# boschresearch/what-matters-for-meta-learning

Hardware: AMD Instinct MI355X
Metric: meta-tasks/sec (fwd+bwd), ANP ShapeNet1D 15+15-shot 16-task batch (higher is better)
Workload: dtype f32

## Files before the change

### what-matters-for-meta-learning_amd/csrc/conv_tc.h

```cpp
#pragma once
#include "common.h"

#ifndef MLHOT_HOSTSIM
namespace mlhot {
#ifdef MLHOT_TS
namespace tf { extern __device__ long long* g_ts_dev; }
#endif
namespace c2 {

typedef float f32x4_t __attribute__((ext_vector_type(4)));

constexpr int CIN = 32, COUT = 48;
constexpr int NT = 768;
#ifndef C12_NT_STORE
#define C12_NT_STORE 0
#endif
#ifndef C12_M1_LANE0
#define C12_M1_LANE0 0
#endif
#ifndef C12_EARLY_PIXELS
#define C12_EARLY_PIXELS 0
#endif
constexpr int RS = 65, ROWS = 9, PS = ROWS * RS;
constexpr int PATCH_FLOATS = CIN * PS;
// ... 199 lines not shown
  return iy1 >= 0 ? (((size_t)img * 64 + iy1) * 4 + cg) * M1_REC : (size_t)n_img * 4096;
}

struct Conv1Tile {
  float a[3];
  f32x4_t c0, c1;
};
__device__ __forceinline__ void c1t_mfma(Conv1Tile& t, const Conv1W& cw, int i) {
  const int ks = i >> 1;
  const f32x4_t zero = {0.f, 0.f, 0.f, 0.f};
  if (i & 1) t.c1 = mfma4(t.a[ks], cw.b[ks][1], ks == 0 ? zero : t.c1);
  else t.c0 = mfma4(t.a[ks], cw.b[ks][0], ks == 0 ? zero : t.c0);
}
template <bool MASK>
__device__ __forceinline__ void c1t_post(Conv1Tile& t, int r, float* d, unsigned* __restrict__ mrec) {
  if (!MASK) {
    d[r] = __int_as_float(max(__float_as_int(t.c0[r]), 0));
    d[16 * PS + r] = __int_as_float(max(__float_as_int(t.c1[r]), 0));
    return;
  }
  const bool p0 = t.c0[r] > 0.f, p1 = t.c1[r] > 0.f;
  d[r] = p0 ? t.c0[r] : 0.f;
  d[16 * PS + r] = p1 ? t.c1[r] : 0.f;
  if (MASK) {
    const unsigned long long b0 = __builtin_amdgcn_ballot_w64(p0), b1 = __builtin_amdgcn_ballot_w64(p1);
    *reinterpret_cast<uint4*>(mrec + 4 * r) = make_uint4((unsigned)b0, (unsigned)(b0 >> 32), (unsigned)b1, (unsigned)(b1 >> 32));
  }
}
constexpr int CS = 34, CROW = RS * CS, CPATCH = ROWS * CROW;
static_assert(2 * CPATCH * 4 <= 160 * 1024, "LDS");
__device__ __forceinline__ float* c1t_dst_cl(float* patch, int t, int lr, int lq) {
  return patch + ((t >> 2) * RS + 1 + 16 * (t & 3) + 4 * lq) * CS + lr;
}
template <bool MASK>
__device__ __forceinline__ void c1t_post_cl(Conv1Tile& t, int r, float* d, unsigned* __restrict__ mrec, bool lane0 = true) {
  const bool p0 = t.c0[r] > 0.f, p1 = t.c1[r] > 0.f;
  d[r * CS] = p0 ? t.c0[r] : 0.f;
  d[r * CS + 16] = p1 ? t.c1[r] : 0.f;
  if (MASK) {
    const unsigned long long b0 = __builtin_amdgcn_ballot_w64(p0), b1 = __builtin_amdgcn_ballot_w64(p1);
#if C12_M1_LANE0
    if (lane0)
#endif
    *reinterpret_cast<uint4*>(mrec + 4 * r) = make_uint4((unsigned)b0, (unsigned)(b0 >> 32), (unsigned)b1, (unsigned)(b1 >> 32));
  }
}
__device__ __forceinline__ void patch_zero_pad_cl(float* patch, int tid) {
  for (int i = tid; i < ROWS * CS; i += NT) patch[(i / CS) * CROW + i % CS] = 0.f;
}

__device__ __forceinline__ float* c1t_dst(float* patch, int t, int lr, int lq) {
  return patch + lr * PS + (t >> 2) * RS + 1 + 16 * (t & 3) + 4 * lq;
}
__device__ __forceinline__ unsigned* c1t_rec(unsigned* __restrict__ m1, int tile, int tt, int n_img) {
  return m1 + m1_record(tile >> 3, 8 * (tile & 7) - 1 + (tt >> 2), tt & 3, n_img);
}
template <bool MASK, bool CL = false>
__device__ __forceinline__ void conv1_tile(const Conv1A& ca, const Conv1W& cw, int j, float* patch, int tile, int wave, int lane,
                                           unsigned* __restrict__ m1, int n_img) {
  const int lr = lane & 15, lq = lane >> 4, tt = wave + 12 * j;
  Conv1Tile t;
#pragma unroll
  for (int ks = 0; ks < 3; ++ks) t.a[ks] = ca.a[j][ks];
#pragma unroll
  for (int i = 0; i < 6; ++i) c1t_mfma(t, cw, i);
  float* d = CL ? c1t_dst_cl(patch, tt, lr, lq) : c1t_dst(patch, tt, lr, lq);
  unsigned* mrec = MASK ? c1t_rec(m1, tile, tt, n_img) : nullptr;
#pragma unroll
  for (int r = 0; r < 4; ++r) {
    if (CL) c1t_post_cl<MASK>(t, r, d, mrec); else c1t_post<MASK>(t, r, d, mrec);
  }
}

__device__ __forceinline__ float strip_line(const ImgSrc& x, int tile, int li) {
  li = min(li, 75);
  const int row = min(max(16 * (tile & 7) - 3 + (li >> 2), 0), 127);
  return x.img(tile >> 3)[row * 128 + 32 * (li & 3)];
}

__global__ __launch_bounds__(NT) void conv12_fwd_pool_kernel(const ImgSrc x, const float* __restrict__ w1, const float* __restrict__ b1,
                                                             const float* __restrict__ w, const float* __restrict__ bias,
                                                             float* __restrict__ p2, uint8_t* __restrict__ amax,
                                                             unsigned* __restrict__ m1, int n_img, int dbg) {
  __shared__ __attribute__((aligned(16))) float patch2[2 * CPATCH];
  static_assert(COUT * W2_LD <= 2 * CPATCH, "weight staging area");
  const int tid = threadIdx.x, lane = tid & 63, wave = __builtin_amdgcn_readfirstlane(tid >> 6);
  const int nt = wave % 3, pg = wave / 3, rp = pg >> 1, ch = pg & 1;
  const int lr = lane & 15, lq = lane >> 4;
  const int n = nt * 16 + lr;
  const int phase = __builtin_amdgcn_readfirstlane(wave >> 2);
#ifdef MLHOT_TS
  if (tf::g_ts_dev && blockIdx.x == 0 && tid == 0) tf::g_ts_dev[502] = clock64();
#endif

  conv2w_stage<NT>(patch2, w, tid);
  __syncthreads();
  float wr[72];
#pragma unroll
  for (int ks = 0; ks < 72; ++ks) wr[ks] = patch2[n * W2_LD + (8 * ((ks & 7) >> 1) + 2 * lq + (ks & 1)) * 9 + (ks >> 3)];
  const float bn = bias[n];
  __syncthreads();
  Conv1W cw;
  conv1w_load(cw, w1, b1, lr, lq);
  Conv1Lane cl;
  conv1lane_init(cl, wave, lr, lq);

  patch_zero_pad_cl(patch2, tid);
  patch_zero_pad_cl(patch2 + CPATCH, tid);
  const int ntiles = n_img * 8;
  int tile = first_tile<8>(blockIdx.x, gridDim.x);
#ifdef MLHOT_TS
  long long ts_c0 = clock64(), ts_w0 = wall_clock64();
  if (tf::g_ts_dev && blockIdx.x == 0 && tid == 0) tf::g_ts_dev[503] = ts_c0;
#endif
  if (tile < ntiles) {
    Conv1A ca;
    conv1a_fetch(ca, x, tile, wave, lr, lq);
#pragma unroll
    for (int j = 0; j < 3; ++j) conv1_tile<true, true>(ca, cw, j, patch2, tile, wave, lane, m1, n_img);
  }
  __syncthreads();
  const int aoff = ((4 * rp) * RS + 2 * (16 * ch + lr)) * CS + 2 * lq;
  int cur = 0;
  float warm = 0.f;
  if (wave < 2 && tile + (int)gridDim.x < ntiles) warm = strip_line(x, tile + (int)gridDim.x, tid);
  for (; tile < ntiles; tile += gridDim.x, cur ^= 1) {
    const float* ab = patch2 + cur * CPATCH + aoff;
    float* nb = patch2 + (cur ^ 1) * CPATCH;
    const int next = tile + (int)gridDim.x < ntiles ? tile + (int)gridDim.x : tile;

#ifdef MLHOT_TS
    const bool tsb = tf::g_ts_dev && blockIdx.x == 0 && (tile - (int)blockIdx.x) / (int)gridDim.x == 6;
    if (tsb && (lane == 0)) tf::g_ts_dev[400 + wave * 4 + 0] = clock64();
#endif
    f32x4_t acc0 = {0.f, 0.f, 0.f, 0.f}, acc1 = {0.f, 0.f, 0.f, 0.f};
    typedef float f32x2_t __attribute__((ext_vector_type(2)));
    constexpr int RDP = 2;
    auto aread = [&](int p, int row2) {
      const int tap = p >> 2, ky = tap / 3, kx = tap % 3, m = p & 3;
      return *reinterpret_cast<const f32x2_t*>(ab + (ky + row2) * CROW + kx * CS + 8 * m);
    };
    f32x2_t xa0[RDP], xa1[RDP];
#pragma unroll
    for (int d = 0; d < RDP; ++d) { xa0[d] = aread(d, 0); xa1[d] = aread(d, 2); }
    Conv1Tile ct;
    float bnw = bn;
#pragma unroll
    for (int ks = 0; ks < 72; ++ks) {
      if (ks % 24 == 0) set_wave_prio((phase + ks / 24) % 3);
      acc0 = mfma4(xa0[(ks >> 1) % RDP][ks & 1], wr[ks], acc0);
      acc1 = mfma4(xa1[(ks >> 1) % RDP][ks & 1], wr[ks], acc1);
      if ((ks & 1) && (ks >> 1) + RDP < 36) { xa0[(ks >> 1) % RDP] = aread((ks >> 1) + RDP, 0); xa1[(ks >> 1) % RDP] = aread((ks >> 1) + RDP, 2); }
      const int j = ks / 22, s = ks - 22 * j;
      if (j < 3) {
        const int tt = wave + 12 * j;
#if C12_EARLY_PIXELS
        if (j == 0 && s < 3) ct.a[s] = conv1a_pixel_load(cl, x, next, 0, s);
        else if (j < 2 && s >= 12 && s < 15) ct.a[s - 12] = conv1a_pixel_load(cl, x, next, j + 1, s - 12);
#else
        if (s < 3) ct.a[s] = conv1a_pixel_load(cl, x, next, j, s);
#endif
        if (s >= 5 && s < 8) ct.a[s - 5] = conv1a_pixel_blend(ct.a[s - 5], cl, next, j, s - 5, wave >> 2);
        else if (s >= 8 && s < 14) c1t_mfma(ct, cw, s - 8);
#ifdef C12_KNOCK_M1
        else if (s >= 15 && s < 19) c1t_post_cl<false>(ct, s - 15, c1t_dst_cl(nb, tt, lr, lq), nullptr);
#else
        else if (s >= 15 && s < 19) c1t_post_cl<true>(ct, s - 15, c1t_dst_cl(nb, tt, lr, lq), c1t_rec(m1, next, tt, n_img), lane == 0);
#endif
      }
      if (ks == 7) bnw = __builtin_fmaf(warm, 0.f, bn);
      if (ks == 48 && wave < 2) warm = strip_line(x, next + (int)gridDim.x < ntiles ? next + (int)gridDim.x : next, tid);
      __builtin_amdgcn_sched_barrier(0);
    }
#ifdef MLHOT_TS
    if (tsb && (lane == 0)) tf::g_ts_dev[400 + wave * 4 + 1] = clock64();
#endif
    const int img = tile >> 3, band = tile & 7;
    float pv[2]; unsigned pa[2];
#pragma unroll
    for (int j = 0; j < 2; ++j) {
      const float c0 = fmaxf(acc0[2 * j] + bnw, 0.f), c1 = fmaxf(acc0[2 * j + 1] + bnw, 0.f);
      const float c2v = fmaxf(acc1[2 * j] + bnw, 0.f), c3 = fmaxf(acc1[2 * j + 1] + bnw, 0.f);
      float best = c0; unsigned which = 0;
      if (c1 > best) { best = c1; which = 1; }
      if (c2v > best) { best = c2v; which = 2; }
      if (c3 > best) { best = c3; which = 3; }
      pv[j] = best; pa[j] = which;
    }
    const size_t o = (((size_t)img * COUT + n) * 16 + 2 * band + rp) * 16 + 8 * ch + 2 * lq;
#if C12_NT_STORE
    __builtin_nontemporal_store(f32x2_t{pv[0], pv[1]}, reinterpret_cast<f32x2_t*>(p2 + o));
    __builtin_nontemporal_store((unsigned short)(pa[0] | (pa[1] << 8)), reinterpret_cast<unsigned short*>(amax + o));
#else
    *reinterpret_cast<float2*>(p2 + o) = make_float2(pv[0], pv[1]);
    *reinterpret_cast<unsigned short*>(amax + o) = (unsigned short)(pa[0] | (pa[1] << 8));
#endif
#ifdef MLHOT_TS
    if (tsb && (lane == 0)) tf::g_ts_dev[400 + wave * 4 + 2] = clock64();
#endif
    __syncthreads();
#ifdef MLHOT_TS
    if (tsb && (lane == 0)) tf::g_ts_dev[400 + wave * 4 + 3] = clock64();
#endif
  }
#ifdef MLHOT_TS
  if (tf::g_ts_dev && blockIdx.x == 0 && threadIdx.x == 0) {
    tf::g_ts_dev[500] = clock64() - ts_c0; tf::g_ts_dev[501] = wall_clock64() - ts_w0;
  }
#endif
}

__device__ __forceinline__ int wg_px(int e) { return (e & 7) + ((e >> 2) & 8); }
__device__ __forceinline__ int wg_pyl(int e) { return (e >> 6) & 1; }
__device__ __forceinline__ int wg_co(int e) { return ((e >> 3) & 3) + 4 * (e >> 7); }
__global__ __launch_bounds__(NT) void conv12_wgrad_kernel(const ImgSrc x, const float* __restrict__ w1, const float* __restrict__ b1,
                                                          const float* __restrict__ dp2, const float* __restrict__ p2,
                                                          const uint8_t* __restrict__ amax, float* __restrict__ slab_w,
                                                          float* __restrict__ slab_b, int n_img, int dbg) {
  __shared__ float lds[PATCH_FLOATS + DYT_FLOATS];
  float* patch = lds;
  float* dyt = lds + PATCH_FLOATS;
  const int tid = threadIdx.x, lane = tid & 63, wave = __builtin_amdgcn_readfirstlane(tid >> 6);
  const int mg = wave % 6, ph = wave / 6;
  const int lr = lane & 15, lq = lane >> 4;
  const bool cact = !(dbg & 1);
  Conv1W cw;
  conv1w_load(cw, w1, b1, lr, lq);

  f32x4_t acc[3][3];
#pragma unroll
  for (int i = 0; i < 3; ++i)
#pragma unroll
    for (int j = 0; j < 3; ++j) acc[i][j] = f32x4_t{0.f, 0.f, 0.f, 0.f};
  float bsum[2] = {0.f, 0.f};

  patch_zero_pad(patch, tid);
  const int ntiles = n_img * 8;
  Conv1A ca;
  float cdp[2], cp[2]; unsigned cam[2];
  auto cells_fetch = [&](int t) {
    const int img = t >> 3, band = t & 7;
#pragma unroll
    for (int j = 0; j < 2; ++j) {
      const int e = tid + j * NT, px = wg_px(e), pyl = wg_pyl(e), co = wg_co(e);
      const size_t o = (((size_t)img * COUT + co) * 16 + 2 * band + pyl) * 16 + px;
      cdp[j] = dp2[o]; cp[j] = p2[o]; cam[j] = amax[o];
    }
  };
  int tile = first_tile<8>(blockIdx.x, gridDim.x);
  Conv1Lane cl;
  conv1lane_init(cl, wave, lr, lq);
  if (tile < ntiles) { if (cact) conv1a_fetch_fast(ca, cl, x, tile, wave); cells_fetch(tile); }
  int aoff[3];
#pragma unroll
  for (int i = 0; i < 3; ++i) {
    const int mt = 3 * mg + i, tap = mt >> 1, ky = tap / 3, kx = tap % 3;
    aoff[i] = (16 * (mt & 1) + lr) * PS + ky * RS + kx + 2 * (8 * lq);
  }
  const int boff = (8 * lq) * DS + lr;

  for (; tile < ntiles; tile += gridDim.x) {
#ifdef MLHOT_TS
    const bool tsb = tf::g_ts_dev && blockIdx.x == 0 && lane == 0 && (tile - first_tile<8>(0, gridDim.x)) / (int)gridDim.x == 6;
#define WG_STAMP(i) do { if (tsb) tf::g_ts_dev[360 + wave * 5 + (i)] = clock64(); } while (0)
#else
#define WG_STAMP(i) do { } while (0)
#endif
    WG_STAMP(0);
    __syncthreads();
    WG_STAMP(1);
    if (cact) {
#pragma unroll
      for (int j = 0; j < 3; ++j) conv1_tile<false>(ca, cw, j, patch, tile, wave, lane, nullptr, n_img);
    }
#pragma unroll
    for (int j = 0; j < 2; ++j) {
      const int e = tid + j * NT, px = wg_px(e), pyl = wg_pyl(e), co = wg_co(e);
      const float g = cp[j] > 0.f ? cdp[j] : 0.f;
      bsum[j] += g;
#pragma unroll
      for (int q = 0; q < 4; ++q)
        dyt[((2 * pyl + (q >> 1)) * 32 + 2 * px + (q & 1)) * DS + co] = (cam[j] == (unsigned)q) ? g : 0.f;
    }
    WG_STAMP(2);
    __syncthreads();
    WG_STAMP(3);
    if (tile + (int)gridDim.x < ntiles) { if (cact) conv1a_fetch_fast(ca, cl, x, tile + gridDim.x, wave); cells_fetch(tile + gridDim.x); }

#pragma unroll
    for (int s = 0; s < 16; ++s) {
      const int orow_l = s >> 3, oxb = s & 7;
      float a[3], b[3];
      const int arow = (2 * (2 * ph + orow_l)) * RS + 2 * oxb;
#pragma unroll
      for (int i = 0; i < 3; ++i) a[i] = patch[aoff[i] + arow];
      const int brow = ((2 * ph + orow_l) * 32 + oxb) * DS;
#pragma unroll
      for (int j = 0; j < 3; ++j) b[j] = dyt[boff + brow + 16 * j];
#pragma unroll
      for (int i = 0; i < 3; ++i)
#pragma unroll
        for (int j = 0; j < 3; ++j) acc[i][j] = mfma4(a[i], b[j], acc[i][j]);
    }
    WG_STAMP(4);
  }

  __syncthreads();
  if (ph == 1) {
#pragma unroll
    for (int i = 0; i < 3; ++i)
#pragma unroll
      for (int j = 0; j < 3; ++j)
#pragma unroll
        for (int r = 0; r < 4; ++r) lds[((mg * 9 + i * 3 + j) * 4 + r) * 64 + lane] = acc[i][j][r];
  }
  __syncthreads();
  if (ph == 0) {
    float* sw = slab_w + (size_t)blockIdx.x * (COUT * CIN * 9 + COUT);
#pragma unroll
    for (int i = 0; i < 3; ++i) {
// ... 250 lines not shown
```

### what-matters-for-meta-learning_amd/csrc/encoder.h

```cpp
#pragma once
#include "common.h"
#include "foreach.h"
#include "igemm.h"
#include "ops_direct.h"
#include "problems.h"
#include "favor.h"
#include "conv_tc.h"
#include "conv_split.h"
#include "conv3_tc.h"
#include "enc_linear.h"
#include "../../include/mlhot.h"

namespace mlhot {

struct Options { int conv2_tc; int tail_fused; int materialize_a1; int dbg; int tail_spec; int conv2_split; int conv3_bwd_merged; };
extern Options g_opt;
enum TailSpec : int {
  TAIL_SPEC_FWD_A = 1,
  TAIL_SPEC_FWD_B = 2,
  TAIL_SPEC_FWD_C = 4,
  TAIL_SPEC_BWD_C = 8,
  TAIL_SPEC_BWD_B = 16,
  TAIL_SPEC_BWD_A = 32,
  TAIL_SPEC_ENC_FOLD = 64,
  TAIL_SPEC_LOSS = 128,
  TAIL_SPEC_BWD_B_SPLIT = 512,
  TAIL_SPEC_BWD_C_WG2 = 1024,
  TAIL_SPEC_BWD_A_WG2 = 2048,
  TAIL_SPEC_WG4 = 4096,
  TAIL_SPEC_DEFAULT = TAIL_SPEC_FWD_A | TAIL_SPEC_FWD_B | TAIL_SPEC_FWD_C | TAIL_SPEC_BWD_C | TAIL_SPEC_BWD_B | TAIL_SPEC_BWD_A |
                      TAIL_SPEC_ENC_FOLD | TAIL_SPEC_LOSS | TAIL_SPEC_BWD_B_SPLIT | TAIL_SPEC_BWD_C_WG2 | TAIL_SPEC_BWD_A_WG2 |
                      TAIL_SPEC_WG4,
};
static_assert(TAIL_SPEC_DEFAULT == 7935, "the numeric values are public: tests, scripts and MLHOT_OPTS pass numbers");
constexpr int C2_GRID = 256;

struct EncSaved {
  float* a1; float* p2; uint8_t* am2; float* a3; unsigned* m1; bool ok; size_t bytes;
};
inline EncSaved enc_saved_carve(int n, void* base, size_t cap) {
  Arena a(base, cap);
  EncSaved s;
  s.a1 = a.take<float>((size_t)n * 32 * 64 * 64);
  s.p2 = a.take<float>((size_t)n * 48 * 16 * 16);
  s.am2 = a.take<uint8_t>((size_t)n * 48 * 16 * 16);
  s.a3 = a.take<float>((size_t)n * 4096);
  s.m1 = a.take<unsigned>((size_t)n * 64 * 64 + 16);
  s.ok = a.ok; s.bytes = a.off + 256;
  return s;
}
inline size_t enc_saved_bytes(int n) { return enc_saved_carve(n, nullptr, 0).bytes; }

inline int enc_lin_split(int n) { (void)n; return 32; }
inline int enc_linw_split(int n) { return n >= 64 ? 4 : 1; }
inline int conv3w_split(int n) { int s = n / 4; return s < 1 ? 1 : (s > 128 ? 128 : s); }
inline int conv2w_split(int n) { int s = n / 2; return s < 1 ? 1 : (s > 240 ? 240 : s); }
inline int conv1w_split(int n) { int s = n * 2; return s > 1024 ? 1024 : s; }

struct EncScratch {
  float* a2;
  float* slab;
  float* dy3;
  float* dp2;
  float* dy1;
  bool ok; size_t bytes;
};
inline size_t enc_slab_floats(int n, int dim_w) {
  size_t m = (size_t)enc_lin_split(n) * n * dim_w;
  size_t v;
  v = (size_t)enc_linw_split(n) * dim_w * 4097; if (v > m) m = v;
  v = (size_t)conv3w_split(n) * 64 * 433;       if (v > m) m = v;
  v = (size_t)conv2w_split(n) * 48 * 289;       if (v > m) m = v;
  v = (size_t)conv1w_split(n) * 32 * 10;        if (v > m) m = v;
  v = (size_t)C2_GRID * (64 * 433 + 48 * 289 + 320) + (size_t)2 * C2_GRID * 48 * 288;     if (v > m) m = v;
  return m;
}
inline EncScratch enc_scratch_carve(int n, int dim_w, void* base, size_t cap) {
  Arena a(base, cap);
  EncScratch s;
  s.slab = a.take<float>(enc_slab_floats(n, dim_w));
  const size_t mark = a.off;
  s.a2 = a.take<float>((size_t)n * 48 * 32 * 32);
  const size_t fwd_end = a.off;
  a.off = mark;
  s.dy3 = a.take<float>((size_t)n * 4096);
  s.dp2 = a.take<float>((size_t)n * 48 * 16 * 16);
  s.dy1 = a.take<float>((size_t)n * 32 * 64 * 64);
  if (fwd_end > a.off) a.off = fwd_end;
  s.ok = a.ok; s.bytes = a.off + 256;
  return s;
}
inline size_t enc_scratch_bytes(int n, int dim_w) { return enc_scratch_carve(n, dim_w, nullptr, 0).bytes; }

#ifndef MLHOT_HOSTSIM
inline int conv12_forward(const c2::ImgSrc& xs, int n, const float* w1, const float* b1, const float* w2, const float* b2,
                          const EncSaved& sv, hipStream_t s) {
  if (g_opt.conv2_split & 1) {
    const int grid2 = n * 16 < C2_GRID ? n * 16 : C2_GRID;
    ProfScope ps("enc.conv12.split", s);
    hipLaunchKernelGGL(c2s::conv12_fwd_split_kernel, dim3(grid2), dim3(c2s::NT), 0, s, xs, w1, b1, w2, b2, sv.p2, sv.am2, sv.m1, n);
  } else {
    const int grid = n * 8 < C2_GRID ? n * 8 : C2_GRID;
    ProfScope ps("enc.conv12", s);
    hipLaunchKernelGGL(c2::conv12_fwd_pool_kernel, dim3(grid), dim3(c2::NT), 0, s, xs, w1, b1, w2, b2, sv.p2, sv.am2, sv.m1, n, g_opt.dbg);
  }
  return check_launch("enc.conv12");
}
constexpr int C12_L2 = 48 * 288, C12_R2 = C12_L2 + 48;
inline int conv12_grid(int n) { return n * 8 < C2_GRID ? n * 8 : C2_GRID; }
template <class Between>
inline int conv12_backward(const c2::ImgSrc& xs, int n, const float* w1, const float* b1, const float* w2, const float* dp2,
                           const EncSaved& sv, float* slab_w, float* slab_b, float* slab_1, hipStream_t s, Between&& between) {
  const int grid = conv12_grid(n);
  if (g_opt.conv2_split & 4) {
    ProfScope ps("enc.bwd.conv12.wgrad.split", s);
    hipLaunchKernelGGL(c2s::conv12_wgrad_split_kernel, dim3(grid), dim3(c2s::NT), 0, s, xs, w1, b1, dp2, sv.p2, sv.am2, slab_w, slab_b, n);
  } else {
    ProfScope ps("enc.bwd.conv12.wgrad", s);
    hipLaunchKernelGGL(c2::conv12_wgrad_kernel, dim3(grid), dim3(c2::NT), 0, s, xs, w1, b1, dp2, sv.p2, sv.am2, slab_w, slab_b, n, g_opt.dbg);
  }
  MLHOT_TRY(check_launch("enc.bwd.conv12.wgrad"));
  MLHOT_TRY(between());
  if (g_opt.conv2_split & 2) {
    ProfScope ps("enc.bwd.conv12.dgrad.split", s);
    hipLaunchKernelGGL(c2s::conv12_dgrad_split_kernel, dim3(grid), dim3(c2s::dg::NT2), 0, s, xs, sv.m1, dp2, sv.p2, sv.am2, w2, slab_1, n);
  } else {
    ProfScope ps("enc.bwd.conv12.dgrad", s);
    hipLaunchKernelGGL(c2::conv12_dgrad_kernel, dim3(grid), dim3(c2::NT2), 0, s, xs, sv.m1, dp2, sv.p2, sv.am2, w2, slab_1, n);
  }
  return check_launch("enc.bwd.conv12.dgrad");
}
#endif

struct EncXFold { const float* slab; const float* bias; int k, n; };
inline int enc_forward(const float* img0, int n0, const float* img1, int n1, const mlhot_enc_params& p, int dim_w,
                       Rows2 feat, void* saved, void* scratch, size_t scratch_bytes, hipStream_t s, EncXFold* xfold = nullptr) {
  if (xfold != nullptr) *xfold = EncXFold{nullptr, nullptr, 0, 0};
  const int n = n0 + n1;
  if (n <= 0) return MLHOT_OK;
  EncSaved sv = enc_saved_carve(n, saved, (size_t)-1 / 2);
  EncScratch sc = enc_scratch_carve(n, dim_w, scratch, scratch_bytes);
  if (!sc.ok) { set_error("enc_vanilla_fwd: scratch too small (%zu < %zu)", scratch_bytes, sc.bytes); return MLHOT_ERR_WORKSPACE; }
  const Src2 x{img0, n0, img1, (size_t)128 * 128};
#ifndef MLHOT_HOSTSIM
  if (g_opt.conv2_tc) {
    if (g_opt.materialize_a1) MLHOT_TRY(run_foreach(Conv1Fwd<Src2>{x, p.w1, p.b1, sv.a1}, (size_t)n * 4096, s, "enc.conv1.debug"));
    MLHOT_TRY(conv12_forward(c2::ImgSrc{img0, n0, img1}, n, p.w1, p.b1, p.w2, p.b2, sv, s));
  } else
#endif
  {
    MLHOT_TRY(run_foreach(Conv1Fwd<Src2>{x, p.w1, p.b1, sv.a1}, (size_t)n * 4096, s, "enc.conv1"));
    typedef ConvFwd<32, 64, 64, 48, Src1> C2;
// ... 207 lines not shown
```

### what-matters-for-meta-learning_amd/csrc/mlhot.hip

```cpp
#include <thread>
#include <stdarg.h>
#include <mutex>

#include "common.h"
#include "foreach.h"
#include "igemm.h"
#include "problems.h"
#include "ops_direct.h"
#include "favor.h"
#include "favor2.h"
#include "prefix.h"
#include "encoder.h"
#include "np_vanilla.h"
#include "conv_rt.h"
#include "ingest.h"
#include "augment.h"
#include "bbb_multi.h"
#include "mt_normal.h"
#include "nt_xent.h"
#include "mlp_chain.h"
#include "resnet_trunk.h"
#include "../../include/mlhot.h"

namespace mlhot {
static thread_local char g_err[512] = "";
void set_error(const char* fmt, ...) {
  va_list ap;
  va_start(ap, fmt);
  vsnprintf(g_err, sizeof(g_err), fmt, ap);
  va_end(ap);
}

Options g_opt = {1, 1, 0, 0, TAIL_SPEC_DEFAULT, 0, 1};
int g_favor2 = 1;
#ifndef MLHOT_HOSTSIM
namespace rt { int g_trunk_fuse34 = 1, g_trunk_dual_dgrad = 1, g_trunk_wg_rows = 128; }
#endif


#ifndef MLHOT_HOSTSIM
int g_side_fold = 0;
static std::mutex g_lane_mu;
static SideLane g_lanes[8];
static int g_nlanes = 0;
SideLane* side_lane(hipStream_t main) {
  if (!g_side_fold) return nullptr;
  std::lock_guard<std::mutex> lk(g_lane_mu);
  for (int i = 0; i < g_nlanes; ++i) if (g_lanes[i].main == main) return &g_lanes[i];
  hipStreamCaptureStatus st = hipStreamCaptureStatusNone;
  if (hipStreamIsCapturing(main, &st) != hipSuccess || st != hipStreamCaptureStatusNone) return nullptr;
  if (g_nlanes == 8) return nullptr;
  SideLane l{};
  l.main = main;
  if (hipStreamCreateWithFlags(&l.side, hipStreamNonBlocking) != hipSuccess) return nullptr;
  if (hipEventCreateWithFlags(&l.ev_fork, hipEventDisableTiming) != hipSuccess || hipEventCreateWithFlags(&l.ev_join, hipEventDisableTiming) != hipSuccess) return nullptr;
  g_lanes[g_nlanes] = l;
  return &g_lanes[g_nlanes++];
}

bool g_prof_on = false;
struct ProfRec { const char* what; hipEvent_t a, b; bool open; };
static ProfRec* g_prof = nullptr;
static int g_prof_cap = 0, g_prof_n = 0;
void prof_record(const char* what, hipStream_t s, bool begin) {
  if (g_prof_n >= g_prof_cap) return;
  if (begin) {
    g_prof[g_prof_n].what = what;
    g_prof[g_prof_n].open = hipEventRecord(g_prof[g_prof_n].a, s) == hipSuccess;
  } else if (g_prof[g_prof_n].open && hipEventRecord(g_prof[g_prof_n].b, s) == hipSuccess) {
    ++g_prof_n;
  }
}
#endif
}

using namespace mlhot;

extern "C" {

int mlhot_version(void) { return MLHOT_ABI_VERSION; }
const char* mlhot_last_error(void) { return g_err; }

int mlhot_set_option(const char* name, int value) {
  if (!strcmp(name, "conv2_tc")) { g_opt.conv2_tc = value; return MLHOT_OK; }
  if (!strcmp(name, "conv2_split")) { g_opt.conv2_split = value; return MLHOT_OK; }
  if (!strcmp(name, "tail_fused")) { g_opt.tail_fused = value; return MLHOT_OK; }
  if (!strcmp(name, "tail_spec")) { g_opt.tail_spec = value; return MLHOT_OK; }
  if (!strcmp(name, "conv3_bwd_merged")) { g_opt.conv3_bwd_merged = value; return MLHOT_OK; }
  if (!strcmp(name, "materialize_a1")) { g_opt.materialize_a1 = value; return MLHOT_OK; }
  if (!strcmp(name, "dbg")) { g_opt.dbg = value; return MLHOT_OK; }
  if (!strcmp(name, "favor2")) { g_favor2 = value; return MLHOT_OK; }
#ifndef MLHOT_HOSTSIM
  if (!strcmp(name, "trunk_dual_dgrad")) { rt::g_trunk_dual_dgrad = value; return MLHOT_OK; }
  if (!strcmp(name, "trunk_wg_rows")) { if (value < 16 || value > 128) { set_error("trunk_wg_rows: 16 .. 128"); return MLHOT_ERR_ARG; } rt::g_trunk_wg_rows = value; return MLHOT_OK; }
  if (!strcmp(name, "trunk_fuse34")) { rt::g_trunk_fuse34 = value; return MLHOT_OK; }
  if (!strcmp(name, "side_fold")) { g_side_fold = value; return MLHOT_OK; }
#endif
  set_error("mlhot_set_option: unknown option %s", name);
  return MLHOT_ERR_ARG;
}

int mlhot_prof_begin(int max_records) {
#ifndef MLHOT_HOSTSIM
  if (g_prof || max_records <= 0) { set_error("prof_begin: already recording, or bad capacity"); return MLHOT_ERR_ARG; }
  g_prof = new ProfRec[max_records];
  int made = 0;
  for (; made < max_records; ++made) {
    g_prof[made].open = false;
    if (hipEventCreate(&g_prof[made].a) != hipSuccess) break;
    if (hipEventCreate(&g_prof[made].b) != hipSuccess) { (void)hipEventDestroy(g_prof[made].a); break; }
  }
  g_prof_cap = made; g_prof_n = 0; g_prof_on = true;
#else
  (void)max_records;
#endif
  return MLHOT_OK;
}
int mlhot_prof_end(const char** labels, float* ms, int cap) {
// ... 576 lines not shown
```

### what-matters-for-meta-learning_amd/mlhot/binding.py

```python
import ctypes as C
import os

import torch

HEADS = 8
MAX_HIDDEN = 4

ACT = {"none": 0, "relu": 1, "tanh": 2}
AGG = {"mean": 0, "max": 1, "baco": 2, "attention": 3}
LOSS = {"azimuth": 0, "mse": 1, "quaternion": 2, "degree": 3, "distractor": 4}

_f = C.c_void_p


ABI_VERSION = 7


AUG_RECORD_BYTES = 128


class MlhotError(RuntimeError):
    pass


# ... 233 lines not shown
        s = EncParams()
        for name, t in zip(("w1", "b1", "w2", "b2", "w3", "b3", "wl", "bl"), tensors):
            setattr(s, name, t.data_ptr())
        return s

    def enc_vanilla_fwd(self, img0, img1, params, dim_w):
        n0 = img0.shape[0]
        n1 = 0 if img1 is None else img1.shape[0]
        _chk(img0, img1, *params)
        n = n0 + n1
        feat0 = torch.empty(n0, dim_w, device=img0.device)
        feat1 = torch.empty(n1, dim_w, device=img0.device)
        saved = self._bytes(self.c.mlhot_enc_vanilla_saved_bytes(n), img0)
        sb = self.c.mlhot_enc_vanilla_scratch_bytes(n, dim_w)
        scratch = self._bytes(sb, img0)
        ps = self.enc_struct(params)
        self._rc(self.c.mlhot_enc_vanilla_fwd(_ptr(img0), n0, _ptr(img1), n1, C.byref(ps), dim_w, _ptr(feat0), dim_w,
                                              _ptr(feat1), dim_w, _ptr(saved), _ptr(scratch), sb, _stream(img0)),
                 "mlhot_enc_vanilla_fwd")
        return feat0, feat1, saved

    def conv12_fwd(self, img, w1, b1, w2, b2):
        _chk(img, w1, b1, w2, b2)
        n = img.shape[0]
        saved = self._bytes(self.c.mlhot_enc_vanilla_saved_bytes(n), img)
        self._rc(self.c.mlhot_conv12_fwd(_ptr(img), n, _ptr(w1), _ptr(b1), _ptr(w2), _ptr(b2), _ptr(saved), _stream(img)),
                 "mlhot_conv12_fwd")
        _, p2, am2, _ = self.enc_saved_views(saved, n)
        return p2, am2, saved

    def conv12_bwd(self, img, w1, b1, w2, dp2, saved):
        _chk(img, w1, b1, w2, dp2)
        n = img.shape[0]
        dw1, db1, dw2 = torch.empty_like(w1), torch.empty_like(b1), torch.empty_like(w2)
        db2 = torch.empty(48, device=img.device)
        sb = self.c.mlhot_conv12_scratch_bytes(n)
        scratch = self._bytes(sb, img)
        self._rc(self.c.mlhot_conv12_bwd(_ptr(img), n, _ptr(w1), _ptr(b1), _ptr(w2), _ptr(dp2), _ptr(saved), _ptr(dw1), _ptr(db1),
                                         _ptr(dw2), _ptr(db2), _ptr(scratch), sb, _stream(img)), "mlhot_conv12_bwd")
        return dw1, db1, dw2, db2

    @staticmethod
    def enc_saved_views(saved, n):
        def al(x):
            return (x + 255) // 256 * 256
        o = 0
        a1 = saved[o:o + n * 32 * 4096 * 4].view(torch.float32).view(n, 32, 64, 64)
        o = al(o + n * 32 * 4096 * 4)
        p2 = saved[o:o + n * 48 * 256 * 4].view(torch.float32).view(n, 48, 16, 16)
        o = al(o + n * 48 * 256 * 4)
        am2 = saved[o:o + n * 48 * 256].view(n, 48, 16, 16)
        o = al(o + n * 48 * 256)
        a3 = saved[o:o + n * 4096 * 4].view(torch.float32).view(n, 64, 8, 8)
        return a1, p2, am2, a3

    @staticmethod
    def enc_routes(saved, n):
        def al(x):
            return (x + 255) // 256 * 256
        _, p2, am2, a3 = MlhotLib.enc_saved_views(saved, n)
        o = al(n * 32 * 4096 * 4)
        o = al(o + n * 48 * 256 * 4)
        o = al(o + n * 48 * 256)
        o = al(o + n * 4096 * 4)
        words = saved[o:o + n * 4096 * 4].view(torch.int32).view(n, 64, 4, 4, 2, 2, 1, 1).cpu()
        shifts = (16 * torch.arange(2, dtype=torch.int32).view(2, 1) + torch.arange(16, dtype=torch.int32).view(1, 16))
        bits = (words >> shifts) & 1
        m1 = bits.permute(0, 4, 7, 1, 2, 5, 6, 3).reshape(n, 32, 64, 64).float()
        return m1, am2.cpu(), (p2 > 0).float().cpu(), (a3 > 0).float().cpu()

    @staticmethod
    def np_saved_views(saved, dims):
        def al(x):
            return (x + 255) // 256 * 256
        Rc, Rq = dims.T * dims.Nc, dims.T * dims.Nq
        n, dw = Rc + Rq, dims.dim_w
        lib = MlhotLib._last
        o = al(lib.c.mlhot_enc_vanilla_saved_bytes(n))

        def take(rows, cols, dtype=torch.float32):
            nonlocal o
            v = saved[o:o + rows * cols * 4].view(dtype).view(rows, cols)
            o = al(o + rows * cols * 4)
            return v
        out = {"enc": saved, "n": n}
        out["dec_in"] = take(Rq, dw + dims.dim_z)
        out["d1"], out["d2"] = take(Rq, dims.dec_hidden), take(Rq, dims.dec_hidden)
        if dims.Nc > 0:
            out["cat_in"] = take(Rc, dw + dw // 4)
            out["h"] = [take(Rc, dims.hidden[i]) for i in range(dims.n_hidden)]
            out["rs"] = take(Rc, dims.dim_r)
            if dims.agg_mode != AGG["attention"]:
                out["r"], out["zt"] = take(dims.T, dims.dim_r), take(dims.T, dims.dim_z)
                out["amax"] = take(dims.T, dims.dim_r, torch.int32)
        return out

    def enc_vanilla_bwd(self, img0, img1, params, dim_w, dfeat0, dfeat1, saved):
        n0 = img0.shape[0]
        n1 = 0 if img1 is None else img1.shape[0]
        _chk(dfeat0, dfeat1)
        grads = [torch.empty_like(p) for p in params]
        sb = self.c.mlhot_enc_vanilla_scratch_bytes(n0 + n1, dim_w)
        scratch = self._bytes(sb, img0)
        ps, gs = self.enc_struct(params), self.enc_struct(grads)
        self._rc(self.c.mlhot_enc_vanilla_bwd(_ptr(img0), n0, _ptr(img1), n1, C.byref(ps), dim_w, _ptr(dfeat0), dim_w,
                                              _ptr(dfeat1), dim_w, _ptr(saved), C.byref(gs), _ptr(scratch), sb, _stream(img0)),
                 "mlhot_enc_vanilla_bwd")
        return grads

    def conv2d_fwd(self, x, w, b, stride, pad, relu):
        _chk(x, w, b)
        N, Cin, H, W = x.shape
        Cout, _, k, _ = w.shape
        HO, WO = (H + 2 * pad - k) // stride + 1, (W + 2 * pad - k) // stride + 1
        y = torch.empty(N, Cout, HO, WO, device=x.device)
        self._rc(self.c.mlhot_conv2d_fwd(_ptr(x), _ptr(w), _ptr(b), _ptr(y), N, Cin, H, W, Cout, k, stride, pad, int(relu), _stream(x)),
                 "mlhot_conv2d_fwd")
        return y

    def conv2d_bwd(self, x, w, y, dy, stride, pad, relu, need_dx=True, has_bias=True):
        _chk(x, w, y, dy)
        N, Cin, H, W = x.shape
        Cout, _, k, _ = w.shape
        dx = torch.empty_like(x) if need_dx else None
        dw = torch.empty_like(w)
        db = torch.empty(Cout, device=x.device) if has_bias else None
        sb = self.c.mlhot_conv2d_bwd_scratch_bytes(N, Cin, H, W, Cout, k, stride, pad)
        scratch = self._bytes(sb, x)
        self._rc(self.c.mlhot_conv2d_bwd(_ptr(x), _ptr(w), _ptr(y), _ptr(dy), N, Cin, H, W, Cout, k, stride, pad, int(relu),
                                         _ptr(dx), _ptr(dw), _ptr(db), _ptr(scratch), sb, _stream(x)), "mlhot_conv2d_bwd")
        return dx, dw, db

    def add_relu_fwd(self, a, b):
# ... 579 lines not shown
        d.agg_mode, d.out_tanh, d.m_feat = AGG[agg_mode], int(out_tanh), m_feat
        return d

    @staticmethod
    def np_struct(cls, dims, tensors, proj=None):
        s = cls()
        pm = vanilla_param_map(dims.n_hidden, dims.agg_mode == AGG["baco"], dims.agg_mode == AGG["attention"])
        for path, key in pm:
            _set(s, path, tensors[key].data_ptr())
        if proj is not None:
            s.proj = proj.data_ptr()
        return s

    def np_vanilla_fwd(self, dims, params, ctx_x, ctx_y, qry_x, proj=None, exchange=None):
        _chk(ctx_x, ctx_y, qry_x, proj, *params.values())
        mu = torch.empty(dims.T, dims.Nq, dims.y_dim, device=qry_x.device)
        saved = self._bytes(self.c.mlhot_np_saved_bytes(C.byref(dims)), qry_x)
        sb = self.c.mlhot_np_scratch_bytes(C.byref(dims))
        scratch = self._bytes(sb, qry_x)
        ps = self.np_struct(NpParams, dims, params, proj)
        if exchange is not None:
            self._staged(lambda st, xp: self._rc(self.c.mlhot_np_vanilla_fwd_staged(
                C.byref(dims), C.byref(ps), _ptr(ctx_x), _ptr(ctx_y), _ptr(qry_x), _ptr(mu), _ptr(saved), _ptr(scratch), sb, st, xp,
                _stream(qry_x)), "mlhot_np_vanilla_fwd_staged"), exchange, "fwd")
            return mu, saved, scratch
        self._rc(self.c.mlhot_np_vanilla_fwd(C.byref(dims), C.byref(ps), _ptr(ctx_x), _ptr(ctx_y), _ptr(qry_x), _ptr(mu),
                                             _ptr(saved), _ptr(scratch), sb, _stream(qry_x)), "mlhot_np_vanilla_fwd")
        return mu, saved, scratch

    def np_vanilla_bwd(self, dims, params, ctx_x, ctx_y, qry_x, mu, dmu, saved, scratch=None, proj=None, exchange=None, loss=None):
        _chk(dmu, mu)
        if loss is not None and exchange is not None:
            raise MlhotError("np_vanilla_bwd: the staged pass takes dmu, not a loss descriptor")
        offs = NpGrads()
        total = self.c.mlhot_np_grads_flat_layout(C.byref(dims), C.byref(offs))
        flat = torch.empty(total, dtype=torch.float32, device=qry_x.device)
        pm = vanilla_param_map(dims.n_hidden, dims.agg_mode == AGG["baco"], dims.agg_mode == AGG["attention"])
        grads = {}
        for path, key in pm:
            off = (_get(offs, path) or 0) // 4
            grads[key] = flat[off:off + params[key].numel()].view_as(params[key])
        sb = self.c.mlhot_np_scratch_bytes(C.byref(dims))
        if scratch is None or scratch.numel() < sb:
            scratch = self._bytes(sb, qry_x)
        ps = self.np_struct(NpParams, dims, params, proj)
        gs = self.np_struct(NpGrads, dims, grads)
        if exchange is not None:
            self._staged(lambda st, xp: self._rc(self.c.mlhot_np_vanilla_bwd_staged(
                C.byref(dims), C.byref(ps), _ptr(ctx_x), _ptr(ctx_y), _ptr(qry_x), _ptr(mu), _ptr(dmu), C.byref(gs), _ptr(saved),
                _ptr(scratch), sb, st, xp, _stream(qry_x)), "mlhot_np_vanilla_bwd_staged"), exchange, "bwd")
            return grads
        if loss is not None:
            kind, gt, dloss, *rest = loss
            value = rest[0] if rest else None
            _chk(gt, dloss)
            if value is not None:
                _chk(value)
            if gt.numel() % (dims.T * dims.Nq) or LOSS[kind] == LOSS["degree"]:
                raise MlhotError(f"np_vanilla_bwd: loss {kind!r} with labels {tuple(gt.shape)} does not fit mu {tuple(mu.shape)}")
            ld = LossDesc(LOSS[kind], _ptr(gt), gt.numel() // (dims.T * dims.Nq), _ptr(dloss), _ptr(value))
            self._rc(self.c.mlhot_np_vanilla_bwd_loss(C.byref(dims), C.byref(ps), _ptr(ctx_x), _ptr(ctx_y), _ptr(qry_x), _ptr(mu), _ptr(dmu),
                                                      C.byref(ld), C.byref(gs), _ptr(saved), _ptr(scratch), sb, _stream(qry_x)), "mlhot_np_vanilla_bwd_loss")
            return grads
        self._rc(self.c.mlhot_np_vanilla_bwd(C.byref(dims), C.byref(ps), _ptr(ctx_x), _ptr(ctx_y), _ptr(qry_x), _ptr(mu), _ptr(dmu),
                                             C.byref(gs), _ptr(saved), _ptr(scratch), sb, _stream(qry_x)), "mlhot_np_vanilla_bwd")
        return grads
# ... 1 lines not shown
```

Baseline: 28650.

## Save conv1 activations in fused forward and reuse them in conv12 weight-gradient

The fused conv1+conv2 forward kernel now also writes post-ReLU conv1 activation tiles to a new global a1s buffer in the saved block. The weight-gradient kernel then loads these tiles instead of recomputing conv1 with MFMAs from the input image. This trades recompute for extra global writes in the forward pass and reads in the backward pass (n*32*64*64 floats), and enlarges the saved memory. The option is on by default, and Python-side checks catch a saved block that is too small.

```diff
diff --git a/what-matters-for-meta-learning_amd/csrc/conv_tc.h b/what-matters-for-meta-learning_amd/csrc/conv_tc.h
--- a/what-matters-for-meta-learning_amd/csrc/conv_tc.h
+++ b/what-matters-for-meta-learning_amd/csrc/conv_tc.h
@@ -255,11 +255,13 @@
 __device__ __forceinline__ float* c1t_dst_cl(float* patch, int t, int lr, int lq) {
   return patch + ((t >> 2) * RS + 1 + 16 * (t & 3) + 4 * lq) * CS + lr;
 }
-template <bool MASK>
+template <bool MASK, bool SAVE = false>
 __device__ __forceinline__ void c1t_post_cl(Conv1Tile& t, int r, float* d, unsigned* __restrict__ mrec, bool lane0 = true) {
   const bool p0 = t.c0[r] > 0.f, p1 = t.c1[r] > 0.f;
-  d[r * CS] = p0 ? t.c0[r] : 0.f;
-  d[r * CS + 16] = p1 ? t.c1[r] : 0.f;
+  const float v0 = p0 ? t.c0[r] : 0.f, v1 = p1 ? t.c1[r] : 0.f;
+  d[r * CS] = v0;
+  d[r * CS + 16] = v1;
+  if (SAVE) { t.c0[r] = v0; t.c1[r] = v1; }
   if (MASK) {
     const unsigned long long b0 = __builtin_amdgcn_ballot_w64(p0), b1 = __builtin_amdgcn_ballot_w64(p1);
 #if C12_M1_LANE0
@@ -272,15 +274,25 @@
   for (int i = tid; i < ROWS * CS; i += NT) patch[(i / CS) * CROW + i % CS] = 0.f;
 }
 
+constexpr int A1S_REC = 2 * 64 * 4;
+constexpr size_t A1S_IMG = (size_t)64 * 4 * A1S_REC;
+__device__ __forceinline__ size_t a1s_record(int tile, int tt) {
+  const int iy1 = 8 * (tile & 7) - 1 + (tt >> 2);
+  return (((size_t)(tile >> 3) * 64 + max(iy1, 0)) * 4 + (tt & 3)) * A1S_REC;
+}
+__device__ __forceinline__ void a1s_store_half(const f32x4_t v, float* __restrict__ a1s, int tile, int tt, int lane, int h) {
+  if (tt >= 4) *reinterpret_cast<f32x4_t*>(a1s + a1s_record(tile, tt) + 256 * h + 4 * lane) = v;
+}
+
 __device__ __forceinline__ float* c1t_dst(float* patch, int t, int lr, int lq) {
   return patch + lr * PS + (t >> 2) * RS + 1 + 16 * (t & 3) + 4 * lq;
 }
 __device__ __forceinline__ unsigned* c1t_rec(unsigned* __restrict__ m1, int tile, int tt, int n_img) {
   return m1 + m1_record(tile >> 3, 8 * (tile & 7) - 1 + (tt >> 2), tt & 3, n_img);
 }
-template <bool MASK, bool CL = false>
+template <bool MASK, bool CL = false, bool SAVE = false>
 __device__ __forceinline__ void conv1_tile(const Conv1A& ca, const Conv1W& cw, int j, float* patch, int tile, int wave, int lane,
-                                           unsigned* __restrict__ m1, int n_img) {
+                                           unsigned* __restrict__ m1, int n_img, float* __restrict__ a1s = nullptr) {
   const int lr = lane & 15, lq = lane >> 4, tt = wave + 12 * j;
   Conv1Tile t;
 #pragma unroll
@@ -291,8 +303,9 @@
   unsigned* mrec = MASK ? c1t_rec(m1, tile, tt, n_img) : nullptr;
 #pragma unroll
   for (int r = 0; r < 4; ++r) {
-    if (CL) c1t_post_cl<MASK>(t, r, d, mrec); else c1t_post<MASK>(t, r, d, mrec);
-  }
+    if (CL) c1t_post_cl<MASK, SAVE>(t, r, d, mrec); else c1t_post<MASK>(t, r, d, mrec);
+  }
+  if (CL && SAVE) { a1s_store_half(t.c0, a1s, tile, tt, lane, 0); a1s_store_half(t.c1, a1s, tile, tt, lane, 1); }
 }
 
 __device__ __forceinline__ float strip_line(const ImgSrc& x, int tile, int li) {
@@ -301,10 +314,11 @@
   return x.img(tile >> 3)[row * 128 + 32 * (li & 3)];
 }
 
+template <bool SAVE>
 __global__ __launch_bounds__(NT) void conv12_fwd_pool_kernel(const ImgSrc x, const float* __restrict__ w1, const float* __restrict__ b1,
                                                              const float* __restrict__ w, const float* __restrict__ bias,
                                                              float* __restrict__ p2, uint8_t* __restrict__ amax,
-                                                             unsigned* __restrict__ m1, int n_img, int dbg) {
+                                                             unsigned* __restrict__ m1, float* __restrict__ a1s, int n_img, int dbg) {
   __shared__ __attribute__((aligned(16))) float patch2[2 * CPATCH];
   static_assert(COUT * W2_LD <= 2 * CPATCH, "weight staging area");
   const int tid = threadIdx.x, lane = tid & 63, wave = __builtin_amdgcn_readfirstlane(tid >> 6);
@@ -340,7 +354,7 @@
     Conv1A ca;
     conv1a_fetch(ca, x, tile, wave, lr, lq);
 #pragma unroll
-    for (int j = 0; j < 3; ++j) conv1_tile<true, true>(ca, cw, j, patch2, tile, wave, lane, m1, n_img);
+    for (int j = 0; j < 3; ++j) conv1_tile<true, true, SAVE>(ca, cw, j, patch2, tile, wave, lane, m1, n_img, a1s);
   }
   __syncthreads();
   const int aoff = ((4 * rp) * RS + 2 * (16 * ch + lr)) * CS + 2 * lq;
@@ -388,8 +402,9 @@
 #ifdef C12_KNOCK_M1
         else if (s >= 15 && s < 19) c1t_post_cl<false>(ct, s - 15, c1t_dst_cl(nb, tt, lr, lq), nullptr);
 #else
-        else if (s >= 15 && s < 19) c1t_post_cl<true>(ct, s - 15, c1t_dst_cl(nb, tt, lr, lq), c1t_rec(m1, next, tt, n_img), lane == 0);
-#endif
+        else if (s >= 15 && s < 19) c1t_post_cl<true, SAVE>(ct, s - 15, c1t_dst_cl(nb, tt, lr, lq), c1t_rec(m1, next, tt, n_img), lane == 0);
+#endif
+        else if (SAVE && s >= 19 && s < 21) a1s_store_half(s == 19 ? ct.c0 : ct.c1, a1s, next, tt, lane, s - 19);
       }
       if (ks == 7) bnw = __builtin_fmaf(warm, 0.f, bn);
       if (ks == 48 && wave < 2) warm = strip_line(x, next + (int)gridDim.x < ntiles ? next + (int)gridDim.x : next, tid);
@@ -436,10 +451,33 @@
 __device__ __forceinline__ int wg_px(int e) { return (e & 7) + ((e >> 2) & 8); }
 __device__ __forceinline__ int wg_pyl(int e) { return (e >> 6) & 1; }
 __device__ __forceinline__ int wg_co(int e) { return ((e >> 3) & 3) + 4 * (e >> 7); }
+struct A1Tiles { f32x4_t c[3][2]; };
+__device__ __forceinline__ void a1s_fetch(A1Tiles& at, const float* __restrict__ a1s, int tile, int wave, int lane) {
+#pragma unroll
+  for (int j = 0; j < 3; ++j) {
+    const float* rec = a1s + a1s_record(tile, wave + 12 * j) + 4 * lane;
+    at.c[j][0] = *reinterpret_cast<const f32x4_t*>(rec);
+    at.c[j][1] = *reinterpret_cast<const f32x4_t*>(rec + 256);
+  }
+}
+__device__ __forceinline__ void a1s_to_patch(const A1Tiles& at, float* patch, int tile, int wave, int lr, int lq) {
+#pragma unroll
+  for (int j = 0; j < 3; ++j) {
+    const int tt = wave + 12 * j;
+    float* d = c1t_dst(patch, tt, lr, lq);
+    const bool keep = j > 0 || (tile & 7) > 0 || tt >= 4;
+#pragma unroll
+    for (int r = 0; r < 4; ++r) {
+      d[r] = keep ? at.c[j][0][r] : 0.f;
+      d[16 * PS + r] = keep ? at.c[j][1][r] : 0.f;
+    }
+  }
+}
+template <bool SAVED>
 __global__ __launch_bounds__(NT) void conv12_wgrad_kernel(const ImgSrc x, const float* __restrict__ w1, const float* __restrict__ b1,
                                                           const float* __restrict__ dp2, const float* __restrict__ p2,
-                                                          const uint8_t* __restrict__ amax, float* __restrict__ slab_w,
-                                                          float* __restrict__ slab_b, int n_img, int dbg) {
+                                                          const uint8_t* __restrict__ amax, const float* __restrict__ a1s,
+                                                          float* __restrict__ slab_w, float* __restrict__ slab_b, int n_img, int dbg) {
   __shared__ float lds[PATCH_FLOATS + DYT_FLOATS];
   float* patch = lds;
   float* dyt = lds + PATCH_FLOATS;
@@ -448,7 +486,7 @@
   const int lr = lane & 15, lq = lane >> 4;
   const bool cact = !(dbg & 1);
   Conv1W cw;
-  conv1w_load(cw, w1, b1, lr, lq);
+  if (!SAVED) conv1w_load(cw, w1, b1, lr, lq);
 
   f32x4_t acc[3][3];
 #pragma unroll
@@ -460,6 +498,7 @@
   patch_zero_pad(patch, tid);
   const int ntiles = n_img * 8;
   Conv1A ca;
+  A1Tiles at;
   float cdp[2], cp[2]; unsigned cam[2];
   auto cells_fetch = [&](int t) {
     const int img = t >> 3, band = t & 7;
@@ -472,8 +511,12 @@
   };
   int tile = first_tile<8>(blockIdx.x, gridDim.x);
   Conv1Lane cl;
-  conv1lane_init(cl, wave, lr, lq);
-  if (tile < ntiles) { if (cact) conv1a_fetch_fast(ca, cl, x, tile, wave); cells_fetch(tile); }
+  if (!SAVED) conv1lane_init(cl, wave, lr, lq);
+  auto a1_fetch = [&](int t) {
+    if (!cact) return;
+    if (SAVED) a1s_fetch(at, a1s, t, wave, lane); else conv1a_fetch_fast(ca, cl, x, t, wave);
+  };
+  if (tile < ntiles) { a1_fetch(tile); cells_fetch(tile); }
   int aoff[3];
 #pragma unroll
   for (int i = 0; i < 3; ++i) {
@@ -493,8 +536,11 @@
     __syncthreads();
     WG_STAMP(1);
     if (cact) {
-#pragma unroll
-      for (int j = 0; j < 3; ++j) conv1_tile<false>(ca, cw, j, patch, tile, wave, lane, nullptr, n_img);
+      if (SAVED) a1s_to_patch(at, patch, tile, wave, lr, lq);
+      else {
+#pragma unroll
+        for (int j = 0; j < 3; ++j) conv1_tile<false>(ca, cw, j, patch, tile, wave, lane, nullptr, n_img);
+      }
     }
 #pragma unroll
     for (int j = 0; j < 2; ++j) {
@@ -508,7 +554,7 @@
     WG_STAMP(2);
     __syncthreads();
     WG_STAMP(3);
-    if (tile + (int)gridDim.x < ntiles) { if (cact) conv1a_fetch_fast(ca, cl, x, tile + gridDim.x, wave); cells_fetch(tile + gridDim.x); }
+    if (tile + (int)gridDim.x < ntiles) { a1_fetch(tile + gridDim.x); cells_fetch(tile + gridDim.x); }
 
 #pragma unroll
     for (int s = 0; s < 16; ++s) {
diff --git a/what-matters-for-meta-learning_amd/csrc/encoder.h b/what-matters-for-meta-learning_amd/csrc/encoder.h
--- a/what-matters-for-meta-learning_amd/csrc/encoder.h
+++ b/what-matters-for-meta-learning_amd/csrc/encoder.h
@@ -13,7 +13,7 @@
 
 namespace mlhot {
 
-struct Options { int conv2_tc; int tail_fused; int materialize_a1; int dbg; int tail_spec; int conv2_split; int conv3_bwd_merged; };
+struct Options { int conv2_tc; int tail_fused; int materialize_a1; int dbg; int tail_spec; int conv2_split; int conv3_bwd_merged; int conv12_save_a1; };
 extern Options g_opt;
 enum TailSpec : int {
   TAIL_SPEC_FWD_A = 1,
@@ -36,8 +36,9 @@
 constexpr int C2_GRID = 256;
 
 struct EncSaved {
-  float* a1; float* p2; uint8_t* am2; float* a3; unsigned* m1; bool ok; size_t bytes;
+  float* a1; float* p2; uint8_t* am2; float* a3; unsigned* m1; float* a1s; bool ok; size_t bytes;
 };
+inline bool conv12_saves_a1() { return g_opt.conv2_tc && g_opt.conv12_save_a1 && !(g_opt.conv2_split & 1); }
 inline EncSaved enc_saved_carve(int n, void* base, size_t cap) {
   Arena a(base, cap);
   EncSaved s;
@@ -46,6 +47,7 @@
   s.am2 = a.take<uint8_t>((size_t)n * 48 * 16 * 16);
   s.a3 = a.take<float>((size_t)n * 4096);
   s.m1 = a.take<unsigned>((size_t)n * 64 * 64 + 16);
+  s.a1s = conv12_saves_a1() ? a.take<float>((size_t)n * 32 * 64 * 64) : nullptr;
   s.ok = a.ok; s.bytes = a.off + 256;
   return s;
 }
@@ -102,7 +104,8 @@
   } else {
     const int grid = n * 8 < C2_GRID ? n * 8 : C2_GRID;
     ProfScope ps("enc.conv12", s);
-    hipLaunchKernelGGL(c2::conv12_fwd_pool_kernel, dim3(grid), dim3(c2::NT), 0, s, xs, w1, b1, w2, b2, sv.p2, sv.am2, sv.m1, n, g_opt.dbg);
+    if (sv.a1s != nullptr) hipLaunchKernelGGL(c2::conv12_fwd_pool_kernel<true>, dim3(grid), dim3(c2::NT), 0, s, xs, w1, b1, w2, b2, sv.p2, sv.am2, sv.m1, sv.a1s, n, g_opt.dbg);
+    else hipLaunchKernelGGL(c2::conv12_fwd_pool_kernel<false>, dim3(grid), dim3(c2::NT), 0, s, xs, w1, b1, w2, b2, sv.p2, sv.am2, sv.m1, nullptr, n, g_opt.dbg);
   }
   return check_launch("enc.conv12");
 }
@@ -117,7 +120,8 @@
     hipLaunchKernelGGL(c2s::conv12_wgrad_split_kernel, dim3(grid), dim3(c2s::NT), 0, s, xs, w1, b1, dp2, sv.p2, sv.am2, slab_w, slab_b, n);
   } else {
     ProfScope ps("enc.bwd.conv12.wgrad", s);
-    hipLaunchKernelGGL(c2::conv12_wgrad_kernel, dim3(grid), dim3(c2::NT), 0, s, xs, w1, b1, dp2, sv.p2, sv.am2, slab_w, slab_b, n, g_opt.dbg);
+    if (sv.a1s != nullptr && !(g_opt.dbg & 4)) hipLaunchKernelGGL(c2::conv12_wgrad_kernel<true>, dim3(grid), dim3(c2::NT), 0, s, xs, w1, b1, dp2, sv.p2, sv.am2, sv.a1s, slab_w, slab_b, n, g_opt.dbg);
+    else hipLaunchKernelGGL(c2::conv12_wgrad_kernel<false>, dim3(grid), dim3(c2::NT), 0, s, xs, w1, b1, dp2, sv.p2, sv.am2, nullptr, slab_w, slab_b, n, g_opt.dbg);
   }
   MLHOT_TRY(check_launch("enc.bwd.conv12.wgrad"));
   MLHOT_TRY(between());
diff --git a/what-matters-for-meta-learning_amd/csrc/mlhot.hip b/what-matters-for-meta-learning_amd/csrc/mlhot.hip
--- a/what-matters-for-meta-learning_amd/csrc/mlhot.hip
+++ b/what-matters-for-meta-learning_amd/csrc/mlhot.hip
@@ -31,7 +31,7 @@
   va_end(ap);
 }
 
-Options g_opt = {1, 1, 0, 0, TAIL_SPEC_DEFAULT, 0, 1};
+Options g_opt = {1, 1, 0, 0, TAIL_SPEC_DEFAULT, 0, 1, 1};
 int g_favor2 = 1;
 #ifndef MLHOT_HOSTSIM
 namespace rt { int g_trunk_fuse34 = 1, g_trunk_dual_dgrad = 1, g_trunk_wg_rows = 128; }
@@ -84,6 +84,7 @@
 int mlhot_set_option(const char* name, int value) {
   if (!strcmp(name, "conv2_tc")) { g_opt.conv2_tc = value; return MLHOT_OK; }
   if (!strcmp(name, "conv2_split")) { g_opt.conv2_split = value; return MLHOT_OK; }
+  if (!strcmp(name, "conv12_save_a1")) { g_opt.conv12_save_a1 = value; return MLHOT_OK; }
   if (!strcmp(name, "tail_fused")) { g_opt.tail_fused = value; return MLHOT_OK; }
   if (!strcmp(name, "tail_spec")) { g_opt.tail_spec = value; return MLHOT_OK; }
   if (!strcmp(name, "conv3_bwd_merged")) { g_opt.conv3_bwd_merged = value; return MLHOT_OK; }
diff --git a/what-matters-for-meta-learning_amd/mlhot/binding.py b/what-matters-for-meta-learning_amd/mlhot/binding.py
--- a/what-matters-for-meta-learning_amd/mlhot/binding.py
+++ b/what-matters-for-meta-learning_amd/mlhot/binding.py
@@ -289,6 +289,7 @@
     def conv12_bwd(self, img, w1, b1, w2, dp2, saved):
         _chk(img, w1, b1, w2, dp2)
         n = img.shape[0]
+        self._chk_saved(saved, self.c.mlhot_enc_vanilla_saved_bytes(n))
         dw1, db1, dw2 = torch.empty_like(w1), torch.empty_like(b1), torch.empty_like(w2)
         db2 = torch.empty(48, device=img.device)
         sb = self.c.mlhot_conv12_scratch_bytes(n)
@@ -296,6 +297,12 @@
         self._rc(self.c.mlhot_conv12_bwd(_ptr(img), n, _ptr(w1), _ptr(b1), _ptr(w2), _ptr(dp2), _ptr(saved), _ptr(dw1), _ptr(db1),
                                          _ptr(dw2), _ptr(db2), _ptr(scratch), sb, _stream(img)), "mlhot_conv12_bwd")
         return dw1, db1, dw2, db2
+
+    @staticmethod
+    def _chk_saved(saved, need):
+        if saved.numel() * saved.element_size() < need:
+            raise MlhotError(f"mlhot: saved block of {saved.numel() * saved.element_size()} bytes, the backward expects {need}: "
+                               "was an option changed between the forward and its backward?")
 
     @staticmethod
     def enc_saved_views(saved, n):
@@ -325,6 +332,20 @@
         bits = (words >> shifts) & 1
         m1 = bits.permute(0, 4, 7, 1, 2, 5, 6, 3).reshape(n, 32, 64, 64).float()
         return m1, am2.cpu(), (p2 > 0).float().cpu(), (a3 > 0).float().cpu()
+
+    @staticmethod
+    def enc_saved_a1(saved, n):
+        def al(x):
+            return (x + 255) // 256 * 256
+        o = al(n * 32 * 4096 * 4)
+        o = al(o + n * 48 * 256 * 4)
+        o = al(o + n * 48 * 256)
+        o = al(o + n * 4096 * 4)
+        o = al(o + (n * 4096 + 16) * 4)
+        if saved.numel() < o + n * 32 * 4096 * 4:
+            raise MlhotError("enc_saved_a1: this saved block has no a1 slot (option conv12_save_a1 off, or not the fused fp32 forward)")
+        rec = saved[o:o + n * 32 * 4096 * 4].view(torch.float32).view(n, 64, 4, 2, 4, 16, 4)
+        return rec.permute(0, 3, 5, 1, 2, 4, 6).reshape(n, 32, 64, 64)
 
     @staticmethod
     def np_saved_views(saved, dims):
@@ -356,6 +377,7 @@
         n0 = img0.shape[0]
         n1 = 0 if img1 is None else img1.shape[0]
         _chk(dfeat0, dfeat1)
+        self._chk_saved(saved, self.c.mlhot_enc_vanilla_saved_bytes(n0 + n1))
         grads = [torch.empty_like(p) for p in params]
         sb = self.c.mlhot_enc_vanilla_scratch_bytes(n0 + n1, dim_w)
         scratch = self._bytes(sb, img0)
@@ -1001,6 +1023,7 @@
         _chk(dmu, mu)
         if loss is not None and exchange is not None:
             raise MlhotError("np_vanilla_bwd: the staged pass takes dmu, not a loss descriptor")
+        self._chk_saved(saved, self.c.mlhot_np_saved_bytes(C.byref(dims)))
         offs = NpGrads()
         total = self.c.mlhot_np_grads_flat_layout(C.byref(dims), C.byref(offs))
         flat = torch.empty(total, dtype=torch.float32, device=qry_x.device)
```

Result: slower. 27560 (-3.8%).
